# shourovrm/binius-NTT

Hardware: AMD Instinct MI355X
Metric: GF(2^128) additive-NTT elements/sec (2^24 pts) (higher is better)
Workload: dtype gf2_128 (u32 limbs, bitwise); 1 GPU; additive NTT over GF(2^128), log_h=24, log_rate=0, one transform per GPU; log_h=24, field=GF(2^128), kernel_variant=5, parallelism=independent transform per rank

## Files before the change

### binius-ntt_amd/csrc/antt_bs.hip

```cpp
#include <hip/hip_runtime.h>

#include <algorithm>
#include <cstdio>
#include <cstring>
#include <type_traits>
#include <vector>

#include "antt_bs.hpp"
#include "antt_bs_dev.hpp"
#include "bitsliced.hpp"
#include "quad_mul.hpp"

namespace bn {

struct BsParams {
	const uint32_t* src;
	uint32_t* dst;
	size_t ntiles;
	int log_h, log_rate;
	unsigned long long* trace;
	int dbg;
	BsPass p;
};

#ifdef BN_DEV
#define BS_DBG(P) ((P).dbg)
#define BS_TRACE(P) ((P).trace != nullptr)
#else
#define BS_DBG(P) 0
#define BS_TRACE(P) false
#endif

template <int L, int ROLE, int FMAX, bool PF>
__device__ __forceinline__ void bs_pass_body(const BsParams& P, size_t tile0) {
	extern __shared__ uint32_t lds[];
	constexpr int NT = 64 * L;
	constexpr bool IN_COMPACT = ROLE == ROLE_FIRST || ROLE == ROLE_SINGLE;
	constexpr bool LAST = ROLE == ROLE_LAST || ROLE == ROLE_SINGLE;
	const BsPass& ps = P.p;
	const int tid = threadIdx.x;
	const int l = tid >> 6, lane = tid & 63;
	uint32_t* plane = lds + l * kPlane;
	uint32_t* cu_w = lds + L * kPlane + l * kMaxStages;
	const size_t n = (size_t)1 << P.log_h;
	const bool TR = BS_TRACE(P);
	unsigned long long tr[8] = {0, 0, 0, 0, 0, 0, 0, 0};
	auto ts = [&]() -> unsigned long long {
		asm volatile("s_waitcnt lgkmcnt(0)" ::: "memory");
		return __builtin_amdgcn_s_memtime();
	};

	auto tile_off = [&](int q) -> size_t {
		size_t off = 0;
#pragma unroll
		for (int m = 0; m < kBlkBits; m++) off |= (size_t)((q >> m) & 1) << ps.bb[m];
		return off;
	};
	size_t outer, outer_off;
	int coset;
	uint32_t* dst;
	const uint32_t* src;
	auto geo = [&](size_t t, size_t& o, size_t& ooff, int& c, uint32_t*& d, const uint32_t*& s) {
		o = t & (((size_t)1 << ps.n_outer) - 1);
		const size_t rest = t >> ps.n_outer;
		c = (int)(rest & ((1u << P.log_rate) - 1));
		const size_t batch = rest >> P.log_rate;
		ooff = 0;
		for (int m = 0; m < ps.n_outer; m++) ooff |= ((o >> m) & 1) << ps.ob[m];
		d = P.dst + (((batch << P.log_rate) + (size_t)c) * n) * L;
		s = IN_COMPACT ? (P.src + batch * n * L) : d;
	};
	uint4 gbuf[kLoads];
	auto issue = [&](const uint32_t* s, size_t ooff) {
#pragma unroll
		for (int r = 0; r < kLoads; r++) {
			if (IN_COMPACT) {
				const int u = tid + r * NT;
				const int q = u / (8 * L), j = u % (8 * L);
				gbuf[r] = (BS_DBG(P) & 1) ? make_uint4(u, j, q, tid) : ld_stream(s + (ooff | tile_off(q)) * L + 4 * j);
			} else {
				const int u = lane + r * 64;
				const int q = u >> 3, j = u & 7;
				gbuf[r] = (BS_DBG(P) & 1) ? make_uint4(u, j, q, tid) : ld_stream(s + (ooff | tile_off(q)) * L + 32 * l + 4 * j);
			}
		}
	};

	auto tile_tw = [&](int j, int q) -> uint32_t {
		uint32_t w = 0;
#pragma unroll
		for (int m = 0; m < kBlkBits; m++) w ^= ps.twt[j][m] & (uint32_t)__builtin_amdgcn_sbfe(q, m, 1);
		return w;
	};

	auto block_stage = [&](int j, int pair) {
		unsigned long long t_a = TR ? ts() : 0;
		const int m = ps.stage_m[j];
		const int qu = ((pair >> m) << (m + 1)) | (pair & ((1 << m) - 1));
		const int qv = qu | (1 << m);
		const uint32_t w = cu_w[j] ^ tile_tw(j, qu);
		uint32_t* pu = plane + qu * kLimbStride;
		uint32_t* pv = plane + qv * kLimbStride;
		uint32_t W[32], V[32], Pr[32], U[32];
#pragma unroll
		for (int i = 0; i < 32; i += 4) *(uint4*)(V + i) = *(const uint4*)(pv + i);
		if (FMAX <= 8) {
#pragma unroll
			for (int i = 0; i < 32; i += 4) *(uint4*)(U + i) = *(const uint4*)(pu + i);
		}
		bool uni = FMAX == 32 && m == kBlkBits - 1 && ps.field[j] == 32 && !(BS_DBG(P) & 4);
#pragma unroll
		for (int mm = 0; mm < kBlkBits - 1; mm++) uni = uni && ps.twt[j][mm] == 0u;
		if (uni) {
			asm volatile("s_waitcnt lgkmcnt(0)" ::: "memory");
			__builtin_amdgcn_sched_barrier(0);
			bsm5_mul_w(V, (uint32_t)__builtin_amdgcn_readfirstlane((int)cu_w[j]), Pr);
			__builtin_amdgcn_sched_barrier(0);
		} else {
#pragma unroll
		for (int i = 0; i < 32; i++) W[i] = (uint32_t)__builtin_amdgcn_sbfe(w, i, 1);
		if (TR) {
			const unsigned long long t = ts();
			tr[5] += t - t_a;
			t_a = t;
		}
		if (BS_DBG(P) & 4) {
#pragma unroll
			for (int i = 0; i < 32; i++) Pr[i] = V[i] ^ W[i];
		} else {
			asm volatile("s_waitcnt lgkmcnt(0)" ::: "memory");
			__builtin_amdgcn_sched_barrier(0);
			mul_tw<FMAX>(ps.field[j], V, W, Pr);
			__builtin_amdgcn_sched_barrier(0);
		}
		}
		if (TR) {
			uint32_t acc = 0;
#pragma unroll
			for (int i = 0; i < 32; i++) acc ^= Pr[i];
			asm volatile("" ::"v"(acc));
			const unsigned long long t = ts();
			tr[6] += t - t_a;
			t_a = t;
		}
#pragma unroll
		for (int i = 0; i < 32; i += 4) {
			uint4 u = FMAX <= 8 ? *(const uint4*)(U + i) : *(const uint4*)(pu + i);
			u.x ^= Pr[i];
			u.y ^= Pr[i + 1];
			u.z ^= Pr[i + 2];
			u.w ^= Pr[i + 3];
			*(uint4*)(pu + i) = u;
			*(uint4*)(pv + i) = make_uint4(V[i] ^ u.x, V[i + 1] ^ u.y, V[i + 2] ^ u.z, V[i + 3] ^ u.w);
		}
		if (TR) tr[7] += ts() - t_a;
	};

	size_t tile = tile0;
	geo(tile, outer, outer_off, coset, dst, src);
	if (PF) issue(src, outer_off);
	for (;;) {
		unsigned long long t0 = TR ? ts() : 0;
		if (IN_COMPACT || LAST) __syncthreads();
		if (!PF) issue(src, outer_off);

		if (lane < ps.k) {
			uint32_t c = 0;
			for (int m = 0; m < ps.n_outer; m++) c ^= ps.two[lane][m] & (0u - (uint32_t)((outer >> m) & 1));
			for (int b = 0; b < P.log_rate; b++) c ^= ps.twc[lane][b] & (0u - (uint32_t)((coset >> b) & 1));
			cu_w[lane] = c;
		}

#pragma unroll
		for (int r = 0; r < kLoads; r++) {
			const uint4 g = gbuf[r];
			if (IN_COMPACT) {
				const int u = tid + r * NT;
				const int q = u / (8 * L), j = u % (8 * L);
				const uint32_t w[4] = {g.x, g.y, g.z, g.w};
#pragma unroll
				for (int t = 0; t < 4; t++) {
					const int word = 4 * j + t;
					lds[(word % L) * kPlane + q * kLimbStride + word / L] = w[t];
				}
			} else {
				const int u = lane + r * 64;
				const int q = u >> 3, j = u & 7;
				*(uint4*)(plane + q * kLimbStride + 4 * j) = g;
			}
		}
		const size_t next = tile + gridDim.x;
		const bool has_next = PF && next < P.ntiles;
		size_t n_outer_v = outer, n_ooff = outer_off;
		int n_coset = coset;
		uint32_t* n_dst = dst;
		const uint32_t* n_src = src;
		if (has_next) {
			geo(next, n_outer_v, n_ooff, n_coset, n_dst, n_src);
			issue(n_src, n_ooff);
		}
		if (IN_COMPACT) {
			__syncthreads();
			for (int q = lane; q < kTileBlocks; q += 64) {
				uint32_t* x = plane + q * kLimbStride;
				uint32_t r[32];
#pragma unroll
				for (int i = 0; i < 32; i += 4) *(uint4*)(r + i) = *(const uint4*)(x + i);
				transpose32(r);
#pragma unroll
				for (int i = 0; i < 32; i += 4) *(uint4*)(x + i) = *(const uint4*)(r + i);
			}
		}
		wave_lds_sync();
		unsigned long long t1 = 0;
		if (TR) {
			t1 = ts();
			tr[0] += t1 - t0;
		}

		const int jlow = max(LAST ? 5 : 0, ps.stop_j);
		for (int j = ps.k - 1; j >= jlow; j--) {
			if (!(BS_DBG(P) & 32)) block_stage(j, lane);
			if (BS_DBG(P) & 64)
				asm volatile("" ::: "memory");
			else
				wave_lds_sync();
		}
		if (TR) {
			const unsigned long long t = ts();
			tr[1] += t - t1;
			t1 = t;
		}

		if (LAST) {
			const int qa = lane, qb = qa | (kTileBlocks / 2);
			uint32_t* pa = plane + qa * kLimbStride;
			uint32_t* pb = plane + qb * kLimbStride;
			for (int s = 4; s >= ((BS_DBG(P) & 16) ? 5 : ps.stop_j); s--) {
				const uint32_t d = vgpr(1u << s);
				const uint32_t um = vgpr(~lane_mask(s));
				const uint32_t cb = cu_w[s] ^ tile_tw(s, qb);
				uint32_t W[32], T[32];
#pragma unroll
				for (int i = 0; i < 32; i += 4) {
					const uint4 a = *(const uint4*)(pa + i), b = *(const uint4*)(pb + i);
					T[i] = __builtin_amdgcn_bitop3_b32(a.x >> d, b.x, um, 0xe4);
					T[i + 1] = __builtin_amdgcn_bitop3_b32(a.y >> d, b.y, um, 0xe4);
					T[i + 2] = __builtin_amdgcn_bitop3_b32(a.z >> d, b.z, um, 0xe4);
					T[i + 3] = __builtin_amdgcn_bitop3_b32(a.w >> d, b.w, um, 0xe4);
				}
#pragma unroll
				for (int i = 0; i < 32; i++) W[i] = ps.pat[s][i] ^ (uint32_t)__builtin_amdgcn_sbfe(cb, i, 1);
				if (BS_DBG(P) & 4) {
#pragma unroll
					for (int i = 0; i < 32; i++) T[i] ^= W[i];
				} else {
					asm volatile("s_waitcnt lgkmcnt(0)" ::: "memory");
					__builtin_amdgcn_sched_barrier(0);
					mul_tw<FMAX>(ps.field[s], T, W, T);
					__builtin_amdgcn_sched_barrier(0);
				}
#pragma unroll
				for (int i = 0; i < 32; i += 4) {
					uint32_t A[4], Bv[4];
					*(uint4*)A = *(const uint4*)(pa + i);
					*(uint4*)Bv = *(const uint4*)(pb + i);
#pragma unroll
					for (int t = 0; t < 4; t++) {
						const uint32_t a = __builtin_amdgcn_bitop3_b32(T[i + t], um, A[t], 0x6a);
						const uint32_t b = __builtin_amdgcn_bitop3_b32(T[i + t] >> d, um, Bv[t], 0x6a);
						A[t] = __builtin_amdgcn_bitop3_b32(a << d, um, a, 0x9a);
						Bv[t] = __builtin_amdgcn_bitop3_b32(b << d, um, b, 0x9a);
					}
					*(uint4*)(pa + i) = *(const uint4*)A;
					*(uint4*)(pb + i) = *(const uint4*)Bv;
				}
			}
#pragma unroll
			for (int h = 0; h < 2; h++) {
				uint32_t* x = h ? pb : pa;
				uint32_t r[32];
#pragma unroll
				for (int i = 0; i < 32; i += 4) *(uint4*)(r + i) = *(const uint4*)(x + i);
				transpose32(r);
#pragma unroll
				for (int i = 0; i < 32; i += 4) *(uint4*)(x + i) = *(const uint4*)(r + i);
			}
			if (TR) {
				const unsigned long long t = ts();
				tr[2] += t - t1;
				t1 = t;
			}
		}

		if (LAST) {
			__syncthreads();
			for (int u = tid; u < kTileBlocks * 8 * L; u += NT) {
				const int q = u / (8 * L), j = u % (8 * L);
				uint32_t w[4];
#pragma unroll
				for (int t = 0; t < 4; t++) {
					const int word = 4 * j + t;
					w[t] = lds[(word % L) * kPlane + q * kLimbStride + word / L];
				}
				if (!(BS_DBG(P) & 2)) st_stream(dst + (outer_off | tile_off(q)) * L + 4 * j, make_uint4(w[0], w[1], w[2], w[3]));
			}
		} else {
#pragma unroll 4
			for (int r = 0; r < kTileBlocks * 8 / 64; r++) {
				const int u = lane + r * 64;
				const int q = u >> 3, j = u & 7;
				const uint4 g = *(const uint4*)(plane + q * kLimbStride + 4 * j);
				if (!(BS_DBG(P) & 2)) st_stream(dst + (outer_off | tile_off(q)) * L + 32 * l + 4 * j, g);
			}
		}
		if (TR) {
			tr[3] += ts() - t1;
			tr[4] += 1;
		}
		if (!PF || !has_next) break;
		tile = next;
		outer = n_outer_v;
		outer_off = n_ooff;
		coset = n_coset;
		dst = n_dst;
		src = n_src;
	}
	if (TR && lane == 0) {
		unsigned long long* o = P.trace + ((size_t)blockIdx.x * (NT / 64) + (tid >> 6)) * 8;
		for (int i = 0; i < 8; i++) o[i] = tr[i];
	}
}

template <int L, int ROLE, int FMAX, bool PF>
__global__ __launch_bounds__(64 * L, 2) void antt_bs_pass(BsParams P) {
	bs_pass_body<L, ROLE, FMAX, PF>(P, blockIdx.x);
}

// ... 284 lines not shown
		p.lo = lo;
		p.k = k;
		std::vector<int> bits;
		if (bottom) {
			for (int b = 5; b < 5 + kBlkBits; b++) bits.push_back(b);
		} else {
			for (int b = 5; (int)bits.size() < kBlkBits - k; b++) bits.push_back(b);
			for (int b = lo; b < lo + k; b++) bits.push_back(b);
		}
		for (int m = 0; m < kBlkBits; m++) p.bb[m] = bits[m];
		p.n_outer = 0;
		for (int b = 5; b < log_h; b++)
			if (std::find(bits.begin(), bits.end(), b) == bits.end()) p.ob[p.n_outer++] = b;
		for (int j = 0; j < k; j++) {
			const int s = lo + j;
			uint32_t acc = 0;
			for (int kk = 0; kk < width - s; kk++) acc |= S(s, kk);
			p.field[j] = acc < 256u ? 8 : acc < 65536u ? 16 : 32;
			p.stage_m[j] = -1;
			for (int m = 0; m < kBlkBits; m++) {
				if (p.bb[m] == s) p.stage_m[j] = m;
				p.twt[j][m] = S(s, p.bb[m] - s - 1);
			}
			for (int m = 0; m < p.n_outer; m++) p.two[j][m] = S(s, p.ob[m] - s - 1);
			for (int c = 0; c < plan->log_rate; c++) p.twc[j][c] = S(s, log_h - 1 - s + c);
			if (s < 5) {
				for (int i = 0; i < 32; i++) {
					uint32_t w = 0;
					for (int b = s + 1; b < 5; b++)
						if ((S(s, b - s - 1) >> i) & 1) w ^= lane_mask(b);
					if ((p.twt[j][kBlkBits - 1] >> i) & 1) w ^= ~lane_mask(s);
					p.pat[s][i] = w;
				}
			}
		}
		return p;
	};
	int bottom_k = kMinLogH;
#ifdef BN_DEV
	if (const char* e = getenv("BN_BOTTOM_K")) bottom_k = std::max(kMinLogH - 1, std::min(kMinLogH, atoi(e)));
#endif
	if (log_h - bottom_k < 1) bottom_k = kMinLogH;
	const int rest = log_h - bottom_k;
	const int n_up = (rest + kBlkBits - 1) / kBlkBits;
	auto gf8_stage = [&](int s) {
		uint32_t acc = 0;
		for (int kk = 0; kk < width - s; kk++) acc |= S(s, kk);
		return acc < 256u;
	};
	int hi = log_h;
	for (int i = 0; i < n_up; i++) {
		const int remaining_up = n_up - i;
		int k = (hi - bottom_k + remaining_up - 1) / remaining_up;
#ifndef BN_UP_EVEN
		if (i == 0 && remaining_up > 1) {
			int g = 0;
			while (g < kBlkBits && hi - g - 1 >= bottom_k && gf8_stage(hi - g - 1)) g++;
			const int min_first = (hi - bottom_k) - (remaining_up - 1) * kBlkBits;
			if (g > k && g >= min_first) k = g;
		BN_DEV_FIRST_K(k, min_first); }
#endif
		passes.push_back(make(hi - k, k, false));
		hi -= k;
	}
	passes.push_back(make(0, bottom_k, true));
	for (size_t i = 0; i < passes.size(); i++) {
		const bool first = i == 0, last = i + 1 == passes.size();
		passes[i].role = first && last ? ROLE_SINGLE : first ? ROLE_FIRST : last ? ROLE_LAST : ROLE_MID;
	}
	return passes;
}

#ifdef BN_DEV
#define BS_KERNEL(R) (pf ? (const void*)antt_bs_pass<L, R, FMAX, true> : (const void*)antt_bs_pass<L, R, FMAX, false>)
#else
#define BS_KERNEL(R) ((void)pf, (const void*)antt_bs_pass<L, R, FMAX, false>)
#endif
template <int L, int FMAX>
static const void* kernel_for_f(int role, bool pf) {
	switch (role) {
		case ROLE_FIRST: return BS_KERNEL(ROLE_FIRST);
		case ROLE_MID: return BS_KERNEL(ROLE_MID);
		case ROLE_LAST: return BS_KERNEL(ROLE_LAST);
		default: return BS_KERNEL(ROLE_SINGLE);
	}
}
#undef BS_KERNEL
static const void* kernel_for(int L, int role, int fmax, bool pf) {
	if (L == 4) return fmax <= 8 ? kernel_for_f<4, 8>(role, pf) : kernel_for_f<4, 32>(role, pf);
	return fmax <= 8 ? kernel_for_f<1, 8>(role, pf) : kernel_for_f<1, 32>(role, pf);
}

static const void* split_kernel_for(int role) {
	switch (role) {
		case ROLE_FIRST: return (const void*)antt_bs3_pass<ROLE_FIRST>;
		case ROLE_MID: return (const void*)antt_bs3_pass<ROLE_MID>;
		case ROLE_LAST: return (const void*)antt_bs3_pass<ROLE_LAST>;
		default: return (const void*)antt_bs3_pass<ROLE_SINGLE>;
	}
}

int pass_fmax(const BsPass& p) {
	int f = 8;
	for (int j = 0; j < p.k; j++) f = std::max(f, p.field[j]);
	return f;
}

static size_t lds_bytes(int L) { return ((size_t)L * kPlane + (size_t)L * kMaxStages) * sizeof(uint32_t); }

bool bs_supports(const bn_antt_plan* plan) {
	return plan->log_h >= kMinLogH && plan->log_h - 5 - kBlkBits <= kMaxOuter && plan->log_rate <= kMaxRateBits;
}

int bs_prepare(bn_antt_plan* plan) {
	for (int L : {1, 4})
		for (int role = 0; role < 4; role++)
			for (int f : {8, 32})
				for (int pf = 0; pf < 2; pf++)
					BN_HIP(hipFuncSetAttribute(kernel_for(L, role, f, pf != 0), hipFuncAttributeMaxDynamicSharedMemorySize,
					                           (int)lds_bytes(L)));
	for (int role = 0; role < 4; role++)
		BN_HIP(hipFuncSetAttribute(split_kernel_for(role), hipFuncAttributeMaxDynamicSharedMemorySize, (int)split_lds_bytes()));
#ifdef BN_DEV
	for (int f0 : {8, 32})
		for (int f1 : {8, 32})
			BN_HIP(hipFuncSetAttribute(persist3_kernel(f0, f1), hipFuncAttributeMaxDynamicSharedMemorySize, (int)lds_bytes(4)));
#endif
	int rc = rr_prepare(plan);
	if (rc != BN_OK) return rc;
	int cus = 0;
	BN_HIP(hipDeviceGetAttribute(&cus, hipDeviceAttributeMultiprocessorCount, plan->device));
	plan->num_cus = std::max(cus, 1);
	plan->variant = 5;
	return BN_OK;
}

const BsPass* bs_passes(bn_antt_plan* plan, size_t* n_passes) {
	if (plan->bs_passes.empty()) {
		const auto ps = plan_passes(plan);
		plan->bs_passes.resize(ps.size() * sizeof(BsPass));
		memcpy(plan->bs_passes.data(), ps.data(), plan->bs_passes.size());
	}
	*n_passes = plan->bs_passes.size() / sizeof(BsPass);
	return (const BsPass*)plan->bs_passes.data();
}

struct BsDevKnobs {
	int pf_mode = 0, dbg = 0, stop_stage = -1, split = -1, mid_pf = -1, rr_last = -1;
	bool persist = true, trace = false;
	size_t max_passes = ~(size_t)0;
};

static BsDevKnobs dev_knobs() {
	BsDevKnobs k;
#ifdef BN_DEV
	if (const char* e = getenv("BN_DEBUG_MAX_PASSES")) k.max_passes = (size_t)atoi(e);
	if (const char* e = getenv("BN_PF")) k.pf_mode = atoi(e);
	if (const char* e = getenv("BN_PERSIST")) k.persist = atoi(e) != 0;
	if (const char* e = getenv("BN_DEBUG_FLAGS")) k.dbg = atoi(e);
	if (const char* e = getenv("BN_DEBUG_STOP_STAGE")) k.stop_stage = atoi(e);
	if (const char* e = getenv("BN_SPLIT")) k.split = atoi(e);
	if (const char* e = getenv("BN_MID_PF")) k.mid_pf = atoi(e);
	if (const char* e = getenv("BN_RR_LAST")) k.rr_last = atoi(e);
	k.trace = getenv("BN_TRACE") != nullptr;
#endif
	return k;
}

static bool use_mid_pf(const bn_antt_plan* plan, const BsPass& pass, size_t ntiles, const BsDevKnobs& kn) {
#ifdef BN_DEV
	if (kn.mid_pf != 1) return false;
	if (plan->variant != 5 || plan->limbs != 4 || pass.role != ROLE_MID || pass_fmax(pass) <= 8) return false;
	RtPass rt;
	if (make_rt(pass, false, &rt) != BN_OK) return false;
	return ntiles >= (size_t)8 * (size_t)plan->num_cus;
#else
	(void)plan, (void)pass, (void)ntiles, (void)kn;
	return false;
// ... 242 lines not shown
```

### binius-ntt_amd/csrc/antt_bs.hpp

```cpp
#pragma once

#include <stdint.h>

#include "antt_plan.hpp"

namespace bn {

constexpr int kBlkBits = 7;
constexpr int kTileBlocks = 1 << kBlkBits;
constexpr int kLimbStride = 36;
constexpr int kMinLogH = kBlkBits + 5;
constexpr int kMaxStages = kBlkBits + 5;
constexpr int kMaxOuter = 32 - 5 - kBlkBits;
constexpr int kMaxRateBits = 8;

enum { ROLE_FIRST = 0, ROLE_MID = 1, ROLE_LAST = 2, ROLE_SINGLE = 3 };

struct BsPass {
	int lo, k, role, n_outer, stop_j;
	int bb[kBlkBits];
	int ob[kMaxOuter];
	int stage_m[kMaxStages];
	int field[kMaxStages];
	uint32_t twt[kMaxStages][kBlkBits];
	uint32_t two[kMaxStages][kMaxOuter];
	uint32_t twc[kMaxStages][kMaxRateBits];
	uint32_t pat[5][32];
};

struct RtPass {
	int lo, k, role, n_outer, mlow;
	int bb[kBlkBits];
	int ob[kMaxOuter];
	int jm[kBlkBits];
	int field_m[kBlkBits];
	int field_s[5];
	uint32_t tau[kBlkBits][6];
	uint32_t tau_iw[5][6];
	uint32_t cb_const[5];
	uint32_t two[kMaxStages][kMaxOuter];
	uint32_t twc[kMaxStages][kMaxRateBits];
	uint32_t pat[5][32];
};

const BsPass* bs_passes(bn_antt_plan* plan, size_t* n_passes);
int pass_fmax(const BsPass& p);
int make_rt(const BsPass& p, bool bottom, RtPass* out);
int rr_prepare(bn_antt_plan* plan);
int rr_launch_pass(bn_antt_plan* plan, int i, const uint32_t* d_in, uint32_t* d_out, size_t batch, hipStream_t st);
const void* rr_pass_kernel(bn_antt_plan* plan, const BsPass& pass);
const void* bs_pass_kernel(bn_antt_plan* plan, int i);
int rr_launch_mid_pf(bn_antt_plan* plan, int i, const uint32_t* d_in, uint32_t* d_out, size_t batch, hipStream_t st);
const void* rr_mid_pf_kernel(const BsPass& pass);

}
```

### binius-ntt_amd/python/binius_ntt_amd/__init__.py

```python
import ctypes
import enum
import os

import numpy as np

_HERE = os.path.dirname(os.path.abspath(__file__))
PKG_ROOT = os.path.dirname(os.path.dirname(_HERE))
LIB_PATH = os.environ.get("BINIUS_NTT_AMD_LIB") or os.path.join(PKG_ROOT, "lib", "libbinius_ntt_amd.so")
HEADER_PATH = os.path.join(os.path.dirname(PKG_ROOT), "include", "binius_ntt_amd.h")

BN_OK, BN_ERR_INVALID, BN_ERR_HIP, BN_ERR_UNSUPPORTED, BN_ERR_ALLOC = 0, 1, 2, 3, 4
_ERRNAMES = {1: "BN_ERR_INVALID", 2: "BN_ERR_HIP", 3: "BN_ERR_UNSUPPORTED", 4: "BN_ERR_ALLOC"}

_lib = None


class BnError(RuntimeError):
    def __init__(self, code, msg):
        super().__init__("%s: %s" % (_ERRNAMES.get(code, code), msg))
        self.code = code


def lib():
    global _lib
    if _lib is not None:
        return _lib
    if not os.path.exists(LIB_PATH):
        raise RuntimeError("libbinius_ntt_amd.so not built (run `make -C binius-ntt_amd` or __graft_entry__.build())")
    try:
        import torch
    except ImportError:
        pass
    L = ctypes.CDLL(LIB_PATH)
    vp, sz, i32, u32p = ctypes.c_void_p, ctypes.c_size_t, ctypes.c_int, ctypes.POINTER(ctypes.c_uint32)
    sig = {
        "bn_last_error": (ctypes.c_char_p, []),
        "bn_version": (ctypes.c_char_p, []),
        "bn_check_gpu_capabilities": (i32, []),
        "bn_antt_plan_create": (i32, [i32, i32, i32, i32, ctypes.POINTER(vp)]),
        "bn_antt_plan_destroy": (i32, [vp]),
        "bn_antt_forward_host": (i32, [vp, vp, sz, vp]),
        "bn_antt_forward_device": (i32, [vp, vp, vp, sz, vp]),
        "bn_antt_inverse_device": (i32, [vp, vp, vp, i32, sz, vp]),
        "bn_antt_inverse_host": (i32, [vp, vp, sz, i32, vp]),
        "bn_antt_get_subspace_evals": (i32, [vp, u32p, sz]),
        "bn_antt_plan_query": (i32, [vp, i32, ctypes.POINTER(ctypes.c_int64)]),
        "bn_antt_plan_set_variant": (i32, [vp, i32]),
        "bn_antt_set_event_timing": (i32, [vp, i32]),
        "bn_antt_get_event_timing": (i32, [vp, ctypes.POINTER(ctypes.c_float), i32, ctypes.POINTER(i32)]),
        "bn_antt_time_passes": (i32, [vp, vp, vp, sz, i32, vp, ctypes.POINTER(ctypes.c_float), i32, ctypes.POINTER(i32)]),
        "bn_antt_pass_kernel_name": (i32, [vp, i32, ctypes.c_char_p, sz]),
        "bn_gf128_mul_device": (i32, [vp, vp, vp, sz, vp]),
        "bn_gf128_mul_bitsliced_device": (i32, [vp, vp, vp, sz, vp]),
        "bn_gf32_mul_device": (i32, [vp, vp, vp, sz, vp]),
        "bn_gf128_mul_repeat_device": (i32, [i32, vp, vp, sz, i32, vp]),
        "bn_bitslice_device": (i32, [vp, sz, i32, vp]),
        "bn_multiply_unrolled": (i32, [i32, u32p, u32p, u32p]),
        "bn_multiply_unrolled_device": (i32, [i32, vp, vp, vp, sz, vp]),
        "bn_mul_binary_tower_32b_simd": (i32, [i32, ctypes.c_uint32, ctypes.c_uint32, u32p]),
        "bn_interleave_32b": (i32, [i32, ctypes.c_uint32, ctypes.c_uint32, u32p, u32p]),
        "bn_xor_adjacent_32b": (i32, [i32, ctypes.c_uint32, u32p]),
        "bn_packed32_device": (i32, [i32, i32, vp, vp, vp, vp, sz, vp]),
        "bn_sumcheck_create": (i32, [i32, i32, i32, i32, u32p, ctypes.POINTER(vp)]),
        "bn_sumcheck_create_device": (i32, [i32, i32, i32, i32, vp, i32, ctypes.POINTER(vp)]),
        "bn_sumcheck_create_staged": (i32, [i32, i32, i32, i32, u32p, ctypes.POINTER(vp)]),
        "bn_sumcheck_prepare": (i32, [vp]),
        "bn_sumcheck_round_messages": (i32, [vp, u32p, u32p]),
        "bn_sumcheck_move_to_next_round": (i32, [vp, u32p]),
        "bn_sumcheck_round": (i32, [vp, ctypes.POINTER(i32)]),
        "bn_sumcheck_set_shard": (i32, [vp, i32, i32]),
        "bn_sumcheck_create_shard_device": (i32, [i32, i32, i32, i32, i32, vp, vp, ctypes.POINTER(vp)]),
        "bn_sumcheck_needs_gather": (i32, [vp, ctypes.POINTER(i32)]),
        "bn_sumcheck_set_message_sink": (i32, [vp, vp]),
        "bn_sumcheck_round_messages_sink": (i32, [vp]),
        "bn_sumcheck_stream": (i32, [vp, ctypes.POINTER(vp)]),
        "bn_sumcheck_export_shard": (i32, [vp, u32p, sz]),
        "bn_sumcheck_import_gathered": (i32, [vp, u32p, sz, i32]),
        "bn_sumcheck_destroy": (i32, [vp]),
        "bn_multilinear_composition_eval": (i32, [i32, i32, i32, i32, u32p, u32p, u32p]),
        "bn_multilinear_composition_eval_device": (i32, [i32, i32, i32, i32, vp, u32p, u32p]),
        "bn_sumcheck_interpolate": (i32, [u32p, i32, u32p, u32p]),
        "bn_bb31_ntt_plan_create": (i32, [i32, ctypes.c_uint32, i32, i32, ctypes.POINTER(vp)]),
        "bn_bb31_ntt_plan_destroy": (i32, [vp]),
        "bn_bb31_ntt_forward_host": (i32, [vp, vp, sz, vp, i32]),
# ... 522 lines not shown
```

### include/binius_ntt_amd.h

```cpp
#ifndef BINIUS_NTT_AMD_H
#define BINIUS_NTT_AMD_H

#include <stddef.h>
#include <stdint.h>

#ifdef __cplusplus
extern "C" {
#endif

enum {
	BN_OK = 0,
	BN_ERR_INVALID = 1,
	BN_ERR_HIP = 2,
	BN_ERR_UNSUPPORTED = 3,
	BN_ERR_ALLOC = 4
};

const char* bn_last_error(void);
const char* bn_version(void);

int bn_check_gpu_capabilities(void);

typedef struct bn_antt_plan bn_antt_plan;

int bn_antt_plan_create(int device, int field_bits, int log_h, int log_rate, bn_antt_plan** plan);
int bn_antt_plan_destroy(bn_antt_plan* plan);

int bn_antt_forward_host(bn_antt_plan* plan, const void* in, size_t in_elems, void* out);

int bn_antt_forward_device(bn_antt_plan* plan, const void* d_in, void* d_out, size_t batch, void* stream);

int bn_antt_inverse_device(bn_antt_plan* plan, const void* d_in, void* d_out, int coset, size_t batch, void* stream);
int bn_antt_inverse_host(bn_antt_plan* plan, const void* in, size_t in_elems, int coset, void* out);

int bn_antt_get_subspace_evals(const bn_antt_plan* plan, uint32_t* out, size_t out_words);

int bn_antt_plan_query(const bn_antt_plan* plan, int what, int64_t* value);
int bn_antt_plan_set_variant(bn_antt_plan* plan, int variant);

int bn_antt_set_event_timing(bn_antt_plan* plan, int enable);
int bn_antt_get_event_timing(bn_antt_plan* plan, float* ms_per_kind, int max_kinds, int* n_kinds);
int bn_antt_time_passes(bn_antt_plan* plan, const void* d_in, void* d_out, size_t batch, int reps,
                        void* stream, float* ms_per_pass, int max_passes, int* n_passes);
int bn_antt_pass_kernel_name(bn_antt_plan* plan, int pass, char* buf, size_t cap);

int bn_gf128_mul_device(const void* d_a, const void* d_b, void* d_out, size_t n, void* stream);
int bn_gf128_mul_bitsliced_device(const void* d_a, const void* d_b, void* d_out, size_t n_blocks, void* stream);
int bn_gf32_mul_device(const void* d_a, const void* d_b, void* d_out, size_t n, void* stream);
int bn_gf128_mul_repeat_device(int kind, void* d_state, const void* d_operand, size_t threads, int iters, void* stream);

int bn_bitslice_device(void* d_buf, size_t n_blocks, int untranspose, void* stream);

int bn_multiply_unrolled(int height, const uint32_t* a, const uint32_t* b, uint32_t* dst);
int bn_multiply_unrolled_device(int height, const void* a, const void* b, void* dst, size_t nblocks, void* stream);
int bn_mul_binary_tower_32b_simd(int height, uint32_t a, uint32_t b, uint32_t* out);
int bn_interleave_32b(int height, uint32_t a, uint32_t b, uint32_t* c, uint32_t* d);
int bn_xor_adjacent_32b(int height, uint32_t a, uint32_t* out);
int bn_packed32_device(int op, int height, const void* a, const void* b, void* c, void* d, size_t n, void* stream);

typedef struct bn_sumcheck bn_sumcheck;

int bn_sumcheck_create(int device, int num_vars, int composition_size, int data_is_transposed,
                       const uint32_t* evals, bn_sumcheck** sc);
int bn_sumcheck_create_staged(int device, int num_vars, int composition_size, int data_is_transposed,
                              const uint32_t* evals, bn_sumcheck** sc);
int bn_sumcheck_prepare(bn_sumcheck* sc);
int bn_sumcheck_create_device(int device, int num_vars, int composition_size, int data_is_transposed,
                              void* d_evals, int take_ownership, bn_sumcheck** sc);
int bn_sumcheck_round_messages(bn_sumcheck* sc, uint32_t* sum, uint32_t* points);
int bn_sumcheck_move_to_next_round(bn_sumcheck* sc, const uint32_t* challenge);
int bn_sumcheck_round(const bn_sumcheck* sc, int* round);
int bn_sumcheck_set_shard(bn_sumcheck* sc, int rank, int world);
int bn_sumcheck_create_shard_device(int device, int num_vars, int composition_size, int rank, int world,
                                    const void* d_local, void* stream, bn_sumcheck** sc);
int bn_sumcheck_needs_gather(const bn_sumcheck* sc, int* flag);
int bn_sumcheck_set_message_sink(bn_sumcheck* sc, void* d_words);
int bn_sumcheck_round_messages_sink(bn_sumcheck* sc);
// ... 37 lines not shown
```

Measured before the change: 23.69 billion elements/s.

## Re-layout last-pass tile so low in-word stages run as plain block butterflies

In the last pass, the bit-sliced plane is transposed across 32-block groups, which turns the five intra-word stages (s<5) into ordinary block-level butterflies. These stages now reuse block_stage with row twiddles (twr) and per-lane patterns (pat_rs), replacing the shift/mask butterfly code. A final transpose restores the element layout, and tile_off is hard-wired to contiguous 32-word offsets for LAST, with an assert on bb. The aim is to remove the shift/bitop3 masking overhead, at the cost of extra strided LDS transposes and possible bank conflicts.

```diff
diff --git a/binius-ntt_amd/csrc/antt_bs.hip b/binius-ntt_amd/csrc/antt_bs.hip
--- a/binius-ntt_amd/csrc/antt_bs.hip
+++ b/binius-ntt_amd/csrc/antt_bs.hip
@@ -1,6 +1,7 @@
 #include <hip/hip_runtime.h>
 
 #include <algorithm>
+#include <cassert>
 #include <cstdio>
 #include <cstring>
 #include <type_traits>
@@ -51,6 +52,7 @@
 	};
 
 	auto tile_off = [&](int q) -> size_t {
+		if (LAST) return (size_t)q << 5;
 		size_t off = 0;
 #pragma unroll
 		for (int m = 0; m < kBlkBits; m++) off |= (size_t)((q >> m) & 1) << ps.bb[m];
@@ -93,12 +95,20 @@
 		return w;
 	};
 
-	auto block_stage = [&](int j, int pair) {
+	auto row_tw = [&](int s, int q) -> uint32_t {
+		uint32_t w = 0;
+#pragma unroll
+		for (int m = 0; m < kBlkBits; m++) w ^= ps.twr[s][m] & (uint32_t)__builtin_amdgcn_sbfe(q, m, 1);
+		return w;
+	};
+
+	auto block_stage = [&](int j, int pair, auto lowc) {
+		constexpr bool LOW = decltype(lowc)::value;
 		unsigned long long t_a = TR ? ts() : 0;
-		const int m = ps.stage_m[j];
+		const int m = LOW ? j : ps.stage_m[j];
 		const int qu = ((pair >> m) << (m + 1)) | (pair & ((1 << m) - 1));
 		const int qv = qu | (1 << m);
-		const uint32_t w = cu_w[j] ^ tile_tw(j, qu);
+		const uint32_t w = cu_w[j] ^ (LOW ? row_tw(j, qu) : tile_tw(j, qu));
 		uint32_t* pu = plane + qu * kLimbStride;
 		uint32_t* pv = plane + qv * kLimbStride;
 		uint32_t W[32], V[32], Pr[32], U[32];
@@ -108,7 +118,7 @@
 #pragma unroll
 			for (int i = 0; i < 32; i += 4) *(uint4*)(U + i) = *(const uint4*)(pu + i);
 		}
-		bool uni = FMAX == 32 && m == kBlkBits - 1 && ps.field[j] == 32 && !(BS_DBG(P) & 4);
+		bool uni = !LOW && FMAX == 32 && m == kBlkBits - 1 && ps.field[j] == 32 && !(BS_DBG(P) & 4);
 #pragma unroll
 		for (int mm = 0; mm < kBlkBits - 1; mm++) uni = uni && ps.twt[j][mm] == 0u;
 		if (uni) {
@@ -118,7 +128,7 @@
 			__builtin_amdgcn_sched_barrier(0);
 		} else {
 #pragma unroll
-		for (int i = 0; i < 32; i++) W[i] = (uint32_t)__builtin_amdgcn_sbfe(w, i, 1);
+		for (int i = 0; i < 32; i++) W[i] = (LOW ? ps.pat_rs[j][i] : 0u) ^ (uint32_t)__builtin_amdgcn_sbfe(w, i, 1);
 		if (TR) {
 			const unsigned long long t = ts();
 			tr[5] += t - t_a;
@@ -220,7 +230,7 @@
 
 		const int jlow = max(LAST ? 5 : 0, ps.stop_j);
 		for (int j = ps.k - 1; j >= jlow; j--) {
-			if (!(BS_DBG(P) & 32)) block_stage(j, lane);
+			if (!(BS_DBG(P) & 32)) block_stage(j, lane, std::false_type());
 			if (BS_DBG(P) & 64)
 				asm volatile("" ::: "memory");
 			else
@@ -233,58 +243,42 @@
 		}
 
 		if (LAST) {
+			{
+				uint32_t* x0 = plane + (32 * (lane >> 5)) * kLimbStride + (lane & 31);
+				uint32_t* x1 = x0 + 64 * kLimbStride;
+				uint32_t r0[32], r1[32];
+#pragma unroll
+				for (int e = 0; e < 32; e++) r0[e] = x0[e * kLimbStride];
+#pragma unroll
+				for (int e = 0; e < 32; e++) r1[e] = x1[e * kLimbStride];
+				transpose32(r0);
+#pragma unroll
+				for (int e = 0; e < 32; e++) x0[e * kLimbStride] = r0[e];
+				transpose32(r1);
+#pragma unroll
+				for (int e = 0; e < 32; e++) x1[e * kLimbStride] = r1[e];
+			}
+			wave_lds_sync();
+			for (int s = 4; s >= ((BS_DBG(P) & 16) ? 5 : ps.stop_j); s--) {
+				block_stage(s, lane, std::true_type());
+				wave_lds_sync();
+			}
 			const int qa = lane, qb = qa | (kTileBlocks / 2);
-			uint32_t* pa = plane + qa * kLimbStride;
-			uint32_t* pb = plane + qb * kLimbStride;
-			for (int s = 4; s >= ((BS_DBG(P) & 16) ? 5 : ps.stop_j); s--) {
-				const uint32_t d = vgpr(1u << s);
-				const uint32_t um = vgpr(~lane_mask(s));
-				const uint32_t cb = cu_w[s] ^ tile_tw(s, qb);
-				uint32_t W[32], T[32];
-#pragma unroll
-				for (int i = 0; i < 32; i += 4) {
-					const uint4 a = *(const uint4*)(pa + i), b = *(const uint4*)(pb + i);
-					T[i] = __builtin_amdgcn_bitop3_b32(a.x >> d, b.x, um, 0xe4);
-					T[i + 1] = __builtin_amdgcn_bitop3_b32(a.y >> d, b.y, um, 0xe4);
-					T[i + 2] = __builtin_amdgcn_bitop3_b32(a.z >> d, b.z, um, 0xe4);
-					T[i + 3] = __builtin_amdgcn_bitop3_b32(a.w >> d, b.w, um, 0xe4);
-				}
-#pragma unroll
-				for (int i = 0; i < 32; i++) W[i] = ps.pat[s][i] ^ (uint32_t)__builtin_amdgcn_sbfe(cb, i, 1);
-				if (BS_DBG(P) & 4) {
-#pragma unroll
-					for (int i = 0; i < 32; i++) T[i] ^= W[i];
-				} else {
-					asm volatile("s_waitcnt lgkmcnt(0)" ::: "memory");
-					__builtin_amdgcn_sched_barrier(0);
-					mul_tw<FMAX>(ps.field[s], T, W, T);
-					__builtin_amdgcn_sched_barrier(0);
-				}
-#pragma unroll
-				for (int i = 0; i < 32; i += 4) {
-					uint32_t A[4], Bv[4];
-					*(uint4*)A = *(const uint4*)(pa + i);
-					*(uint4*)Bv = *(const uint4*)(pb + i);
-#pragma unroll
-					for (int t = 0; t < 4; t++) {
-						const uint32_t a = __builtin_amdgcn_bitop3_b32(T[i + t], um, A[t], 0x6a);
-						const uint32_t b = __builtin_amdgcn_bitop3_b32(T[i + t] >> d, um, Bv[t], 0x6a);
-						A[t] = __builtin_amdgcn_bitop3_b32(a << d, um, a, 0x9a);
-						Bv[t] = __builtin_amdgcn_bitop3_b32(b << d, um, b, 0x9a);
-					}
-					*(uint4*)(pa + i) = *(const uint4*)A;
-					*(uint4*)(pb + i) = *(const uint4*)Bv;
-				}
-			}
-#pragma unroll
-			for (int h = 0; h < 2; h++) {
-				uint32_t* x = h ? pb : pa;
-				uint32_t r[32];
-#pragma unroll
-				for (int i = 0; i < 32; i += 4) *(uint4*)(r + i) = *(const uint4*)(x + i);
-				transpose32(r);
-#pragma unroll
-				for (int i = 0; i < 32; i += 4) *(uint4*)(x + i) = *(const uint4*)(r + i);
+			uint32_t ra[32], rb[32];
+#pragma unroll
+			for (int i = 0; i < 32; i += 4) {
+				*(uint4*)(ra + i) = *(const uint4*)(plane + qa * kLimbStride + i);
+				*(uint4*)(rb + i) = *(const uint4*)(plane + qb * kLimbStride + i);
+			}
+			wave_lds_sync();
+			transpose32(ra);
+			transpose32(rb);
+			uint32_t* xa = plane + (qa & ~31) * kLimbStride + (qa & 31);
+			uint32_t* xb = plane + (qb & ~31) * kLimbStride + (qb & 31);
+#pragma unroll
+			for (int e = 0; e < 32; e++) {
+				xa[e * kLimbStride] = ra[e];
+				xb[e * kLimbStride] = rb[e];
 			}
 			if (TR) {
 				const unsigned long long t = ts();
@@ -654,6 +648,15 @@
 					if ((p.twt[j][kBlkBits - 1] >> i) & 1) w ^= ~lane_mask(s);
 					p.pat[s][i] = w;
 				}
+				if (bottom) {
+					for (int m = 0; m < kBlkBits; m++) p.twr[s][m] = m < 5 ? S(s, m - s - 1) : p.twt[j][m];
+					for (int i = 0; i < 32; i++) {
+						uint32_t w = 0;
+						for (int b = 0; b < 5; b++)
+							if ((p.twt[j][b] >> i) & 1) w ^= lane_mask(b);
+						p.pat_rs[s][i] = w;
+					}
+				}
 			}
 		}
 		return p;
@@ -686,6 +689,7 @@
 		hi -= k;
 	}
 	passes.push_back(make(0, bottom_k, true));
+	for (int m = 0; m < kBlkBits; m++) assert(passes.back().bb[m] == 5 + m);
 	for (size_t i = 0; i < passes.size(); i++) {
 		const bool first = i == 0, last = i + 1 == passes.size();
 		passes[i].role = first && last ? ROLE_SINGLE : first ? ROLE_FIRST : last ? ROLE_LAST : ROLE_MID;
diff --git a/binius-ntt_amd/csrc/antt_bs.hpp b/binius-ntt_amd/csrc/antt_bs.hpp
--- a/binius-ntt_amd/csrc/antt_bs.hpp
+++ b/binius-ntt_amd/csrc/antt_bs.hpp
@@ -26,6 +26,8 @@
 	uint32_t two[kMaxStages][kMaxOuter];
 	uint32_t twc[kMaxStages][kMaxRateBits];
 	uint32_t pat[5][32];
+	uint32_t twr[5][kBlkBits];
+	uint32_t pat_rs[5][32];
 };
 
 struct RtPass {
```

Measured after the change: 23.87 billion elements/s (median of 6 runs). Within noise of the previous version (+0.7%).

## Run low in-word NTT stages in packed layout and simplify last-pass addressing

Applied to the files above, without the earlier changes.

In the last pass, the five low butterfly stages that sit inside a 32-bit word now run on a packed pair layout. A pack step is applied first, and each stage fuses its butterfly with the repacking for the next stage using precomputed pat2 twiddle patterns. This replaces the separate per-stage extract, multiply and merge loop, and the final transpose writes the output words straight into their interleaved positions. Global loads and stores in the last pass use contiguous offsets from a base pointer, relying on a new host check that the tile block bits map to index bits 5..11. The change adds the pat2 table to BsParams, a debug export function, and a plan-time failure when that layout assumption does not hold.

```diff
diff --git a/binius-ntt_amd/csrc/antt_bs.hip b/binius-ntt_amd/csrc/antt_bs.hip
--- a/binius-ntt_amd/csrc/antt_bs.hip
+++ b/binius-ntt_amd/csrc/antt_bs.hip
@@ -26,10 +26,13 @@
 #ifdef BN_DEV
 #define BS_DBG(P) ((P).dbg)
 #define BS_TRACE(P) ((P).trace != nullptr)
+#define BS_PACKED(P) (!((P).dbg & 16) && (P).p.stop_j == 0)
 #else
 #define BS_DBG(P) 0
 #define BS_TRACE(P) false
+#define BS_PACKED(P) true
 #endif
+static_assert(sizeof(BsParams) <= 4096, "BsParams is a kernel argument");
 
 template <int L, int ROLE, int FMAX, bool PF>
 __device__ __forceinline__ void bs_pass_body(const BsParams& P, size_t tile0) {
@@ -72,16 +75,19 @@
 	};
 	uint4 gbuf[kLoads];
 	auto issue = [&](const uint32_t* s, size_t ooff) {
+		const uint32_t* const s0 = s + ooff * L;
 #pragma unroll
 		for (int r = 0; r < kLoads; r++) {
 			if (IN_COMPACT) {
 				const int u = tid + r * NT;
 				const int q = u / (8 * L), j = u % (8 * L);
-				gbuf[r] = (BS_DBG(P) & 1) ? make_uint4(u, j, q, tid) : ld_stream(s + (ooff | tile_off(q)) * L + 4 * j);
+				const uint32_t* g = LAST ? s0 + (uint32_t)(4 * u) : s + (ooff | tile_off(q)) * L + 4 * j;
+				gbuf[r] = (BS_DBG(P) & 1) ? make_uint4(u, j, q, tid) : ld_stream(g);
 			} else {
 				const int u = lane + r * 64;
 				const int q = u >> 3, j = u & 7;
-				gbuf[r] = (BS_DBG(P) & 1) ? make_uint4(u, j, q, tid) : ld_stream(s + (ooff | tile_off(q)) * L + 32 * l + 4 * j);
+				const uint32_t* g = LAST ? s0 + (uint32_t)(q * 32 * L + 32 * l + 4 * j) : s + (ooff | tile_off(q)) * L + 32 * l + 4 * j;
+				gbuf[r] = (BS_DBG(P) & 1) ? make_uint4(u, j, q, tid) : ld_stream(g);
 			}
 		}
 	};
@@ -93,9 +99,10 @@
 		return w;
 	};
 
-	auto block_stage = [&](int j, int pair) {
-		unsigned long long t_a = TR ? ts() : 0;
-		const int m = ps.stage_m[j];
+	auto block_stage = [&](int j, int pair, bool inw) {
+		const bool TRB = TR && !inw;
+		unsigned long long t_a = TRB ? ts() : 0;
+		const int m = inw ? kBlkBits - 1 : ps.stage_m[j];
 		const int qu = ((pair >> m) << (m + 1)) | (pair & ((1 << m) - 1));
 		const int qv = qu | (1 << m);
 		const uint32_t w = cu_w[j] ^ tile_tw(j, qu);
@@ -108,7 +115,7 @@
 #pragma unroll
 			for (int i = 0; i < 32; i += 4) *(uint4*)(U + i) = *(const uint4*)(pu + i);
 		}
-		bool uni = FMAX == 32 && m == kBlkBits - 1 && ps.field[j] == 32 && !(BS_DBG(P) & 4);
+		bool uni = FMAX == 32 && !inw && m == kBlkBits - 1 && ps.field[j] == 32 && !(BS_DBG(P) & 4);
 #pragma unroll
 		for (int mm = 0; mm < kBlkBits - 1; mm++) uni = uni && ps.twt[j][mm] == 0u;
 		if (uni) {
@@ -117,9 +124,14 @@
 			bsm5_mul_w(V, (uint32_t)__builtin_amdgcn_readfirstlane((int)cu_w[j]), Pr);
 			__builtin_amdgcn_sched_barrier(0);
 		} else {
-#pragma unroll
-		for (int i = 0; i < 32; i++) W[i] = (uint32_t)__builtin_amdgcn_sbfe(w, i, 1);
-		if (TR) {
+		if (inw) {
+#pragma unroll
+			for (int i = 0; i < 32; i++) W[i] = ps.pat2[j][i] ^ (uint32_t)__builtin_amdgcn_sbfe(w, i, 1);
+		} else {
+#pragma unroll
+			for (int i = 0; i < 32; i++) W[i] = (uint32_t)__builtin_amdgcn_sbfe(w, i, 1);
+		}
+		if (TRB) {
 			const unsigned long long t = ts();
 			tr[5] += t - t_a;
 			t_a = t;
@@ -134,7 +146,7 @@
 			__builtin_amdgcn_sched_barrier(0);
 		}
 		}
-		if (TR) {
+		if (TRB) {
 			uint32_t acc = 0;
 #pragma unroll
 			for (int i = 0; i < 32; i++) acc ^= Pr[i];
@@ -143,17 +155,51 @@
 			tr[6] += t - t_a;
 			t_a = t;
 		}
+		if (inw && j > 0) {
+			const uint32_t d = vgpr(1u << (j - 1));
+			const uint32_t um = vgpr(~lane_mask(j - 1));
+#pragma unroll
+			for (int i = 0; i < 32; i += 4) {
+				uint32_t Uw[4], X[4], Y[4];
+				*(uint4*)Uw = FMAX <= 8 ? *(const uint4*)(U + i) : *(const uint4*)(pu + i);
+#pragma unroll
+				for (int t = 0; t < 4; t++) {
+					const uint32_t x = Uw[t] ^ Pr[i + t], y = V[i + t] ^ x;
+					X[t] = __builtin_amdgcn_bitop3_b32(x, y << d, um, 0xe4);
+					Y[t] = __builtin_amdgcn_bitop3_b32(x >> d, y, um, 0xe4);
+				}
+				*(uint4*)(pu + i) = *(const uint4*)X;
+				*(uint4*)(pv + i) = *(const uint4*)Y;
+			}
+		} else {
+#pragma unroll
+			for (int i = 0; i < 32; i += 4) {
+				uint4 u = FMAX <= 8 ? *(const uint4*)(U + i) : *(const uint4*)(pu + i);
+				u.x ^= Pr[i];
+				u.y ^= Pr[i + 1];
+				u.z ^= Pr[i + 2];
+				u.w ^= Pr[i + 3];
+				*(uint4*)(pu + i) = u;
+				*(uint4*)(pv + i) = make_uint4(V[i] ^ u.x, V[i + 1] ^ u.y, V[i + 2] ^ u.z, V[i + 3] ^ u.w);
+			}
+		}
+		if (TRB) tr[7] += ts() - t_a;
+	};
+	auto pack_pair = [&](uint32_t* pa, uint32_t* pb) {
+		const uint32_t d = vgpr(16u), um = vgpr(~lane_mask(4));
 #pragma unroll
 		for (int i = 0; i < 32; i += 4) {
-			uint4 u = FMAX <= 8 ? *(const uint4*)(U + i) : *(const uint4*)(pu + i);
-			u.x ^= Pr[i];
-			u.y ^= Pr[i + 1];
-			u.z ^= Pr[i + 2];
-			u.w ^= Pr[i + 3];
-			*(uint4*)(pu + i) = u;
-			*(uint4*)(pv + i) = make_uint4(V[i] ^ u.x, V[i + 1] ^ u.y, V[i + 2] ^ u.z, V[i + 3] ^ u.w);
-		}
-		if (TR) tr[7] += ts() - t_a;
+			uint32_t A[4], Bv[4], X[4], Y[4];
+			*(uint4*)A = *(const uint4*)(pa + i);
+			*(uint4*)Bv = *(const uint4*)(pb + i);
+#pragma unroll
+			for (int t = 0; t < 4; t++) {
+				X[t] = __builtin_amdgcn_bitop3_b32(A[t], Bv[t] << d, um, 0xe4);
+				Y[t] = __builtin_amdgcn_bitop3_b32(A[t] >> d, Bv[t], um, 0xe4);
+			}
+			*(uint4*)(pa + i) = *(const uint4*)X;
+			*(uint4*)(pb + i) = *(const uint4*)Y;
+		}
 	};
 
 	size_t tile = tile0;
@@ -218,73 +264,96 @@
 			tr[0] += t1 - t0;
 		}
 
-		const int jlow = max(LAST ? 5 : 0, ps.stop_j);
+		const bool packed = ROLE == ROLE_LAST && BS_PACKED(P);
+		const int qa = lane, qb = qa | (kTileBlocks / 2);
+		uint32_t* pa = plane + qa * kLimbStride;
+		uint32_t* pb = plane + qb * kLimbStride;
+		const int jlow = packed ? 0 : max(LAST ? 5 : 0, ps.stop_j);
 		for (int j = ps.k - 1; j >= jlow; j--) {
-			if (!(BS_DBG(P) & 32)) block_stage(j, lane);
+			const bool inw = packed && j < 5;
+			if (packed && j == 4) {
+				if (TR) {
+					const unsigned long long t = ts();
+					tr[1] += t - t1;
+					t1 = t;
+				}
+				pack_pair(pa, pb);
+			}
+			if (inw || !(BS_DBG(P) & 32)) block_stage(j, lane, inw);
 			if (BS_DBG(P) & 64)
 				asm volatile("" ::: "memory");
 			else
 				wave_lds_sync();
 		}
-		if (TR) {
+		if (TR && !packed) {
 			const unsigned long long t = ts();
 			tr[1] += t - t1;
 			t1 = t;
 		}
 
 		if (LAST) {
-			const int qa = lane, qb = qa | (kTileBlocks / 2);
-			uint32_t* pa = plane + qa * kLimbStride;
-			uint32_t* pb = plane + qb * kLimbStride;
-			for (int s = 4; s >= ((BS_DBG(P) & 16) ? 5 : ps.stop_j); s--) {
-				const uint32_t d = vgpr(1u << s);
-				const uint32_t um = vgpr(~lane_mask(s));
-				const uint32_t cb = cu_w[s] ^ tile_tw(s, qb);
-				uint32_t W[32], T[32];
-#pragma unroll
-				for (int i = 0; i < 32; i += 4) {
-					const uint4 a = *(const uint4*)(pa + i), b = *(const uint4*)(pb + i);
-					T[i] = __builtin_amdgcn_bitop3_b32(a.x >> d, b.x, um, 0xe4);
-					T[i + 1] = __builtin_amdgcn_bitop3_b32(a.y >> d, b.y, um, 0xe4);
-					T[i + 2] = __builtin_amdgcn_bitop3_b32(a.z >> d, b.z, um, 0xe4);
-					T[i + 3] = __builtin_amdgcn_bitop3_b32(a.w >> d, b.w, um, 0xe4);
+			if (packed) {
+				uint32_t X[32], Y[32];
+#pragma unroll
+				for (int i = 0; i < 32; i += 4) *(uint4*)(X + i) = *(const uint4*)(pa + i);
+#pragma unroll
+				for (int i = 0; i < 32; i += 4) *(uint4*)(Y + i) = *(const uint4*)(pb + i);
+				transpose32(X);
+				transpose32(Y);
+#pragma unroll
+				for (int r = 0; r < 32; r += 2)
+					*(uint4*)((r & 16 ? pb : pa) + 2 * (r & 15)) = make_uint4(X[r], Y[r], X[r + 1], Y[r + 1]);
+			} else {
+				for (int s = 4; s >= ((BS_DBG(P) & 16) ? 5 : ps.stop_j); s--) {
+					const uint32_t d = vgpr(1u << s);
+					const uint32_t um = vgpr(~lane_mask(s));
+					const uint32_t cb = cu_w[s] ^ tile_tw(s, qb);
+					uint32_t W[32], T[32];
+#pragma unroll
+					for (int i = 0; i < 32; i += 4) {
+						const uint4 a = *(const uint4*)(pa + i), b = *(const uint4*)(pb + i);
+						T[i] = __builtin_amdgcn_bitop3_b32(a.x >> d, b.x, um, 0xe4);
+						T[i + 1] = __builtin_amdgcn_bitop3_b32(a.y >> d, b.y, um, 0xe4);
+						T[i + 2] = __builtin_amdgcn_bitop3_b32(a.z >> d, b.z, um, 0xe4);
+						T[i + 3] = __builtin_amdgcn_bitop3_b32(a.w >> d, b.w, um, 0xe4);
+					}
+#pragma unroll
+					for (int i = 0; i < 32; i++) W[i] = ps.pat[s][i] ^ (uint32_t)__builtin_amdgcn_sbfe(cb, i, 1);
+					if (BS_DBG(P) & 4) {
+#pragma unroll
+						for (int i = 0; i < 32; i++) T[i] ^= W[i];
+					} else {
+						asm volatile("s_waitcnt lgkmcnt(0)" ::: "memory");
+						__builtin_amdgcn_sched_barrier(0);
+						mul_tw<FMAX>(ps.field[s], T, W, T);
+						__builtin_amdgcn_sched_barrier(0);
+					}
+#pragma unroll
+					for (int i = 0; i < 32; i += 4) {
+						uint32_t A[4], Bv[4];
+						*(uint4*)A = *(const uint4*)(pa + i);
+						*(uint4*)Bv = *(const uint4*)(pb + i);
+#pragma unroll
+						for (int t = 0; t < 4; t++) {
+							const uint32_t a = __builtin_amdgcn_bitop3_b32(T[i + t], um, A[t], 0x6a);
+							const uint32_t b = __builtin_amdgcn_bitop3_b32(T[i + t] >> d, um, Bv[t], 0x6a);
+							A[t] = __builtin_amdgcn_bitop3_b32(a << d, um, a, 0x9a);
+							Bv[t] = __builtin_amdgcn_bitop3_b32(b << d, um, b, 0x9a);
+						}
+						*(uint4*)(pa + i) = *(const uint4*)A;
+						*(uint4*)(pb + i) = *(const uint4*)Bv;
+					}
 				}
 #pragma unroll
-				for (int i = 0; i < 32; i++) W[i] = ps.pat[s][i] ^ (uint32_t)__builtin_amdgcn_sbfe(cb, i, 1);
-				if (BS_DBG(P) & 4) {
-#pragma unroll
-					for (int i = 0; i < 32; i++) T[i] ^= W[i];
-				} else {
-					asm volatile("s_waitcnt lgkmcnt(0)" ::: "memory");
-					__builtin_amdgcn_sched_barrier(0);
-					mul_tw<FMAX>(ps.field[s], T, W, T);
-					__builtin_amdgcn_sched_barrier(0);
+				for (int h = 0; h < 2; h++) {
+					uint32_t* x = h ? pb : pa;
+					uint32_t r[32];
+#pragma unroll
+					for (int i = 0; i < 32; i += 4) *(uint4*)(r + i) = *(const uint4*)(x + i);
+					transpose32(r);
+#pragma unroll
+					for (int i = 0; i < 32; i += 4) *(uint4*)(x + i) = *(const uint4*)(r + i);
 				}
-#pragma unroll
-				for (int i = 0; i < 32; i += 4) {
-					uint32_t A[4], Bv[4];
-					*(uint4*)A = *(const uint4*)(pa + i);
-					*(uint4*)Bv = *(const uint4*)(pb + i);
-#pragma unroll
-					for (int t = 0; t < 4; t++) {
-						const uint32_t a = __builtin_amdgcn_bitop3_b32(T[i + t], um, A[t], 0x6a);
-						const uint32_t b = __builtin_amdgcn_bitop3_b32(T[i + t] >> d, um, Bv[t], 0x6a);
-						A[t] = __builtin_amdgcn_bitop3_b32(a << d, um, a, 0x9a);
-						Bv[t] = __builtin_amdgcn_bitop3_b32(b << d, um, b, 0x9a);
-					}
-					*(uint4*)(pa + i) = *(const uint4*)A;
-					*(uint4*)(pb + i) = *(const uint4*)Bv;
-				}
-			}
-#pragma unroll
-			for (int h = 0; h < 2; h++) {
-				uint32_t* x = h ? pb : pa;
-				uint32_t r[32];
-#pragma unroll
-				for (int i = 0; i < 32; i += 4) *(uint4*)(r + i) = *(const uint4*)(x + i);
-				transpose32(r);
-#pragma unroll
-				for (int i = 0; i < 32; i += 4) *(uint4*)(x + i) = *(const uint4*)(r + i);
 			}
 			if (TR) {
 				const unsigned long long t = ts();
@@ -295,15 +364,22 @@
 
 		if (LAST) {
 			__syncthreads();
-			for (int u = tid; u < kTileBlocks * 8 * L; u += NT) {
-				const int q = u / (8 * L), j = u % (8 * L);
+			uint32_t* const g0 = dst + outer_off * L;
+			const int q0 = tid / (8 * L), j0 = tid % (8 * L);
+			const uint32_t* sp[4];
+#pragma unroll
+			for (int t = 0; t < 4; t++) {
+				const int word = 4 * j0 + t;
+				sp[t] = lds + (word % L) * kPlane + q0 * kLimbStride + word / L;
+			}
+			constexpr int kStoreIters = kTileBlocks * 8 * L / NT;
+			constexpr int kStepBlocks = NT / (8 * L);
+#pragma unroll
+			for (int it = 0; it < kStoreIters; it++) {
 				uint32_t w[4];
 #pragma unroll
-				for (int t = 0; t < 4; t++) {
-					const int word = 4 * j + t;
-					w[t] = lds[(word % L) * kPlane + q * kLimbStride + word / L];
-				}
-				if (!(BS_DBG(P) & 2)) st_stream(dst + (outer_off | tile_off(q)) * L + 4 * j, make_uint4(w[0], w[1], w[2], w[3]));
+				for (int t = 0; t < 4; t++) w[t] = sp[t][it * kStepBlocks * kLimbStride];
+				if (!(BS_DBG(P) & 2)) st_stream(g0 + (uint32_t)(4 * (tid + it * NT)), make_uint4(w[0], w[1], w[2], w[3]));
 			}
 		} else {
 #pragma unroll 4
@@ -654,6 +730,13 @@
 					if ((p.twt[j][kBlkBits - 1] >> i) & 1) w ^= ~lane_mask(s);
 					p.pat[s][i] = w;
 				}
+				for (int i = 0; i < 32; i++) {
+					uint32_t w = 0;
+					for (int b = s + 1; b < 5; b++)
+						if ((S(s, b - s - 1) >> i) & 1) w ^= lane_mask(b - 1);
+					if ((p.twt[j][kBlkBits - 1] >> i) & 1) w ^= lane_mask(4);
+					p.pat2[s][i] = w;
+				}
 			}
 		}
 		return p;
@@ -722,6 +805,12 @@
 	}
 }
 
+static bool bottom_tile_contiguous(const BsPass& p) {
+	for (int m = 0; m < kBlkBits; m++)
+		if (p.bb[m] != 5 + m) return false;
+	return true;
+}
+
 int pass_fmax(const BsPass& p) {
 	int f = 8;
 	for (int j = 0; j < p.k; j++) f = std::max(f, p.field[j]);
@@ -748,6 +837,10 @@
 		for (int f1 : {8, 32})
 			BN_HIP(hipFuncSetAttribute(persist3_kernel(f0, f1), hipFuncAttributeMaxDynamicSharedMemorySize, (int)lds_bytes(4)));
 #endif
+	size_t n_passes = 0;
+	const BsPass* passes = bs_passes(plan, &n_passes);
+	if (n_passes == 0 || !bottom_tile_contiguous(passes[n_passes - 1]))
+		BN_FAIL(BN_ERR_UNSUPPORTED, "bottom pass: tile block bits are not index bits 5..11");
 	int rc = rr_prepare(plan);
 	if (rc != BN_OK) return rc;
 	int cus = 0;
@@ -766,6 +859,42 @@
 	*n_passes = plan->bs_passes.size() / sizeof(BsPass);
 	return (const BsPass*)plan->bs_passes.data();
 }
+
+}
+
+extern "C" int bn_antt_inword_tables(int log_h, int log_rate, uint32_t* out, size_t out_words) {
+	using namespace bn;
+	constexpr size_t kStageWords = 32 + kBlkBits + kMaxOuter + kMaxRateBits + 1;
+	constexpr size_t kWords = 4 + 1 + kMaxOuter + 5 * kStageWords;
+	BN_CHECK_ARG(out != nullptr, "output pointer is NULL");
+	BN_CHECK_ARG(log_rate >= 0 && log_rate <= 4 && log_h + log_rate <= 32, "log_h + log_rate must be <= 32, log_rate in [0,4]");
+	BN_CHECK_ARG(out_words >= kWords, "output holds %zu words, need %zu", out_words, kWords);
+	bn_antt_plan plan;
+	plan.log_h = log_h;
+	plan.log_rate = log_rate;
+	plan.width = log_h + log_rate - 1;
+	if (!bs_supports(&plan)) BN_FAIL(BN_ERR_UNSUPPORTED, "the bitsliced passes need log_h >= %d", kMinLogH);
+	subspace_evals(log_h, log_rate, plan.s_host);
+	const BsPass p = plan_passes(&plan).back();
+	if (!bottom_tile_contiguous(p)) BN_FAIL(BN_ERR_UNSUPPORTED, "bottom pass: tile block bits are not index bits 5..11");
+	uint32_t* o = out;
+	*o++ = (uint32_t)kWords;
+	*o++ = (uint32_t)kBlkBits;
+	*o++ = (uint32_t)kMaxOuter;
+	*o++ = (uint32_t)kMaxRateBits;
+	*o++ = (uint32_t)p.n_outer;
+	for (int m = 0; m < kMaxOuter; m++) *o++ = (uint32_t)p.ob[m];
+	for (int s = 0; s < 5; s++) {
+		for (int i = 0; i < 32; i++) *o++ = p.pat2[s][i];
+		for (int m = 0; m < kBlkBits; m++) *o++ = p.twt[s][m];
+		for (int m = 0; m < kMaxOuter; m++) *o++ = p.two[s][m];
+		for (int c = 0; c < kMaxRateBits; c++) *o++ = p.twc[s][c];
+		*o++ = (uint32_t)p.field[s];
+	}
+	return BN_OK;
+}
+
+namespace bn {
 
 struct BsDevKnobs {
 	int pf_mode = 0, dbg = 0, stop_stage = -1, split = -1, mid_pf = -1, rr_last = -1;
diff --git a/binius-ntt_amd/csrc/antt_bs.hpp b/binius-ntt_amd/csrc/antt_bs.hpp
--- a/binius-ntt_amd/csrc/antt_bs.hpp
+++ b/binius-ntt_amd/csrc/antt_bs.hpp
@@ -26,6 +26,7 @@
 	uint32_t two[kMaxStages][kMaxOuter];
 	uint32_t twc[kMaxStages][kMaxRateBits];
 	uint32_t pat[5][32];
+	uint32_t pat2[5][32];
 };
 
 struct RtPass {
diff --git a/binius-ntt_amd/python/binius_ntt_amd/__init__.py b/binius-ntt_amd/python/binius_ntt_amd/__init__.py
--- a/binius-ntt_amd/python/binius_ntt_amd/__init__.py
+++ b/binius-ntt_amd/python/binius_ntt_amd/__init__.py
@@ -50,6 +50,7 @@
         "bn_antt_get_event_timing": (i32, [vp, ctypes.POINTER(ctypes.c_float), i32, ctypes.POINTER(i32)]),
         "bn_antt_time_passes": (i32, [vp, vp, vp, sz, i32, vp, ctypes.POINTER(ctypes.c_float), i32, ctypes.POINTER(i32)]),
         "bn_antt_pass_kernel_name": (i32, [vp, i32, ctypes.c_char_p, sz]),
+        "bn_antt_inword_tables": (i32, [i32, i32, u32p, sz]),
         "bn_gf128_mul_device": (i32, [vp, vp, vp, sz, vp]),
         "bn_gf128_mul_bitsliced_device": (i32, [vp, vp, vp, sz, vp]),
         "bn_gf32_mul_device": (i32, [vp, vp, vp, sz, vp]),
diff --git a/include/binius_ntt_amd.h b/include/binius_ntt_amd.h
--- a/include/binius_ntt_amd.h
+++ b/include/binius_ntt_amd.h
@@ -43,6 +43,7 @@
 int bn_antt_time_passes(bn_antt_plan* plan, const void* d_in, void* d_out, size_t batch, int reps,
                         void* stream, float* ms_per_pass, int max_passes, int* n_passes);
 int bn_antt_pass_kernel_name(bn_antt_plan* plan, int pass, char* buf, size_t cap);
+int bn_antt_inword_tables(int log_h, int log_rate, uint32_t* out, size_t out_words);
 
 int bn_gf128_mul_device(const void* d_a, const void* d_b, void* d_out, size_t n, void* stream);
 int bn_gf128_mul_bitsliced_device(const void* d_a, const void* d_b, void* d_out, size_t n_blocks, void* stream);
```

After: 23.74 billion elements/s before, 24.30 billion elements/s after, median of 6. 2.4% higher.
